# nv-legate/legate.sparse

Measured on AMD Instinct MI355X. Metric: cg_iters_per_sec, higher is better.
Workload: dtype fp64; 1 GPU; model=poisson2d-5pt-cg, nx=16384, n=268435456, nnz=1342111744, parallelism=dp1 1-D row partition + window gather

## Files before the change

sparse/kernels/__init__.py:

```python
from __future__ import annotations

import os

import torch

_EXT = None
_TRIED = False

_DIR = os.path.dirname(os.path.abspath(__file__))
BUILD_DIR = os.path.join(_DIR, "_build")
SO_PATH = os.path.join(BUILD_DIR, "sparse_hip.so")


def ext():
    global _EXT, _TRIED
    if _EXT is not None or _TRIED:
        return _EXT
    _TRIED = True
    if os.path.exists(SO_PATH):
        torch.ops.load_library(SO_PATH)
        _EXT = torch.ops.sparse_hip
    return _EXT


# ... 392 lines not shown
            and os.environ.get("SPARSE_DIA_NOCOMPRESS") != "1"):
        cvals = torch.zeros(W, dtype=dvals.dtype, device=A.device)
        mdt = (torch.uint8 if W <= 8 else
               torch.uint16 if W <= 16 else torch.uint32)
        mask = torch.empty(mp, dtype=mdt, device=A.device)
        ok = torch.ones(1, dtype=torch.int32, device=A.device)
        ext().dia_classify(dvals, cvals, mask, ok, W)
        if int(ok.item()):
            dvals = None
        else:
            cvals = mask = None
    ho = offs.tolist()
    adj = sum(1 << i for i in range(min(W, 32) - 1) if ho[i + 1] == ho[i] + 1)
    return DiaMirror(dvals, offs, W, m, row0, off_min=ho[0], off_max=ho[-1],
                     cvals=cvals, mask=mask, adj=adj)


def _pieces(p):
    hlo, own, hhi = p
    return hlo.contiguous(), own.contiguous(), hhi.contiguous()


def dia_spmv(dm: DiaMirror, pieces, y, col_lo: int, wsize: int,
             rbase: int = 0, rhi: int = -1):
    ext().dia_spmv(*dm.source(), dm.offs, *_pieces(pieces), y, dm.W, dm.m,
                   int(col_lo), dm.row0, int(wsize), int(rbase), int(rhi),
                   dm.adj)


def dia_spmv_dot(dm: DiaMirror, pieces, y, p, col_lo: int, wsize: int,
                 rbase: int = 0, rhi: int = -1):
    return ext().dia_spmv_dot(*dm.source(), dm.offs, *_pieces(pieces), y, p,
                              dm.W, dm.m, int(col_lo), dm.row0, int(wsize),
                              int(rbase), int(rhi), dm.adj)


def dia_spmv_bpdot(dm: DiaMirror, r_pieces, p_pieces, pnew, q,
                   beta_num, beta_den, col_lo: int, wsize: int):
    return ext().dia_spmv_bpdot(*dm.source(), dm.offs, *_pieces(r_pieces),
                                *_pieces(p_pieces), pnew, q, beta_num,
                                beta_den, dm.W, dm.m, int(col_lo), dm.row0,
                                int(wsize), dm.adj)


def cg_xr_norm2(x, p, r, q, a, b, *, nt: int = -1):
    n = x.numel()
    if n == 0:
        return torch.zeros((), dtype=x.dtype, device=x.device)
    ept = max(1, 16 // x.element_size())
    blocks = (n // ept + 255) // 256 + 1
    partial = torch.empty(blocks, dtype=x.dtype, device=x.device)
    ext().cg_xr_norm2(x, p, r, q, a.to(x.dtype), b.to(x.dtype), partial,
                      int(nt))
    return partial.sum()


def dia_residual(dm: DiaMirror, pieces, b, y, col_lo: int, wsize: int,
# ... 144 lines not shown
```

sparse/kernels/src/common.h:

```cpp
#pragma once

#include <type_traits>

#include <hip/hip_runtime.h>

#include <ATen/ATen.h>
#include <ATen/Dispatch.h>
#include <ATen/hip/HIPContext.h>
#include <c10/util/complex.h>

#define SPARSE_CHECK_HIP(cmd)                                             \
  do {                                                                    \
    hipError_t e = (cmd);                                                 \
    TORCH_CHECK(e == hipSuccess, "HIP error: ", hipGetErrorString(e));    \
  } while (0)

constexpr int WAVE = 64;

__device__ __forceinline__ int64_t ub_i64(const int64_t* arr, int64_t n, int64_t key) {
  int64_t lo = 0, hi = n;
  while (lo < hi) {
    int64_t mid = (lo + hi) >> 1;
    if (arr[mid] <= key) lo = mid + 1; else hi = mid;
  }
// ... 71 lines not shown
    if (lane == 0) ws[n * NW + wid] = s;
  }
  __syncthreads();
  T s = ZeroOf<T>::value();
  if (threadIdx.x < N) {
    const T* w = ws + threadIdx.x * NW;
    s = ((w[0] + w[1]) + w[2]) + w[3];
  }
  return s;
}

inline hipStream_t cur_stream() {
  return c10::hip::getCurrentHIPStreamMasqueradingAsCUDA().stream();
}

template <typename T>
__device__ __forceinline__ T nt_load(const T* __restrict__ p) {
  if constexpr (std::is_arithmetic_v<T>) {
    return __builtin_nontemporal_load(p);
  } else {
    return *p;
  }
}
```

sparse/kernels/src/elemwise.hip:

```cpp
#include "common.h"

namespace {

template <typename index_t>
__global__ void add_nnz_kernel(const int64_t* __restrict__ aip,
                               const index_t* __restrict__ aix,
                               const int64_t* __restrict__ bip,
                               const index_t* __restrict__ bix,
                               int64_t* __restrict__ out, int64_t m) {
  int64_t r = (int64_t)blockIdx.x * blockDim.x + threadIdx.x;
  if (r >= m) return;
  int64_t pa = aip[r], ea = aip[r + 1];
  int64_t pb = bip[r], eb = bip[r + 1];
  int64_t c = 0;
  while (pa < ea && pb < eb) {
    index_t ca = aix[pa], cb = bix[pb];
    if (ca == cb) { ++pa; ++pb; }
    else if (ca < cb) ++pa;
    else ++pb;
    ++c;
  }
  out[r] = c + (ea - pa) + (eb - pb);
}

// ... 98 lines not shown
    static_assert(sizeof(VVec<T>) == 16, "non-temporal path moves 16 bytes");
    const u32x4_t t =
        __builtin_nontemporal_load(reinterpret_cast<const u32x4_t*>(p));
    VVec<T> v;
    __builtin_memcpy(&v, &t, 16);
    return v;
  } else {
    return *p;
  }
}

template <bool NT, typename T>
__device__ __forceinline__ void vec_store(VVec<T>* p, const VVec<T>& v) {
  if constexpr (NT) {
    static_assert(sizeof(VVec<T>) == 16, "non-temporal path moves 16 bytes");
    u32x4_t t;
    __builtin_memcpy(&t, &v, 16);
    __builtin_nontemporal_store(t, reinterpret_cast<u32x4_t*>(p));
  } else {
    *p = v;
  }
}

enum : int { NT_NONE = 0, NT_READS = 1, NT_ALL = 2 };

template <typename T, bool ISALPHA, bool NEG, int NT>
__global__ __launch_bounds__(256) void axpby_kernel(
    T* __restrict__ y, const T* __restrict__ x, const T* __restrict__ a,
    const T* __restrict__ b, int64_t n) {
  constexpr int EPT = EptOf<T>::value;
  T s = (*a) / (*b);
  if (NEG) s = -s;
  const int64_t nv = n / EPT;
  const int64_t i = (int64_t)blockIdx.x * blockDim.x + threadIdx.x;
  if (i < nv) {
    auto* y2 = reinterpret_cast<VVec<T>*>(y);
    auto* x2 = reinterpret_cast<const VVec<T>*>(x);
    VVec<T> yv = vec_load<NT == NT_ALL>(y2 + i);
    const VVec<T> xv = vec_load<NT != NT_NONE>(x2 + i);
#pragma unroll
    for (int j = 0; j < EPT; ++j) {
      yv.v[j] = ISALPHA ? (yv.v[j] + s * xv.v[j]) : (xv.v[j] + s * yv.v[j]);
    }
    vec_store<NT == NT_ALL>(y2 + i, yv);
  }
  if (blockIdx.x == 0 && threadIdx.x == 0) {
    for (int64_t t = nv * EPT; t < n; ++t) {
      y[t] = ISALPHA ? (y[t] + s * x[t]) : (x[t] + s * y[t]);
    }
  }
}

constexpr int kStreamNtAuto = NT_ALL;
constexpr int64_t kStreamNtMinBytes = int64_t(256) << 20;

inline int stream_nt_mode(int64_t nt, int64_t vec_bytes, const char* who) {
  TORCH_CHECK(nt >= -1 && nt <= 2, who, ": nt must be -1, 0, 1 or 2, got ", nt);
  if (nt >= 0) return (int)nt;
  return vec_bytes >= kStreamNtMinBytes ? kStreamNtAuto : NT_NONE;
}

}

void add_nnz_hip(at::Tensor aip, at::Tensor aix, at::Tensor bip, at::Tensor bix,
                 at::Tensor out) {
  int64_t m = out.numel();
  if (m == 0) return;
  DISPATCH_INDEX(aix.scalar_type(), "add_nnz", [&] {
    hipLaunchKernelGGL((add_nnz_kernel<index_t>), dim3((m + 255) / 256), dim3(256),
                       0, cur_stream(), aip.data_ptr<int64_t>(),
                       aix.data_ptr<index_t>(), bip.data_ptr<int64_t>(),
                       bix.data_ptr<index_t>(), out.data_ptr<int64_t>(), m);
  });
  SPARSE_CHECK_HIP(hipGetLastError());
}

void add_compute_hip(at::Tensor aip, at::Tensor aix, at::Tensor av,
                     at::Tensor bip, at::Tensor bix, at::Tensor bv,
                     at::Tensor cip, at::Tensor cix, at::Tensor cv,
                     double alpha, double beta) {
  int64_t m = aip.numel() - 1;
  if (m == 0) return;
// ... 219 lines not shown
```

sparse/kernels/src/ops.cpp:

```cpp
#include <algorithm>

#include <torch/library.h>

#include <ATen/ATen.h>

void spmv_hip(at::Tensor, at::Tensor, at::Tensor, at::Tensor, at::Tensor,
              int64_t, double);
void spmv_dot_hip(at::Tensor, at::Tensor, at::Tensor, at::Tensor, at::Tensor,
                  at::Tensor, at::Tensor, int64_t);
void axpby_norm2_hip(at::Tensor, at::Tensor, at::Tensor, at::Tensor, bool,
                     bool, at::Tensor);
void build_ell_hip(at::Tensor, at::Tensor, at::Tensor, at::Tensor, at::Tensor,
                   int64_t, int64_t);
void build_dia_hip(at::Tensor, at::Tensor, at::Tensor, at::Tensor, at::Tensor,
                   int64_t, int64_t);
void ell_spmv_plain_hip(at::Tensor, at::Tensor, at::Tensor, at::Tensor,
                        at::Tensor, at::Tensor, int64_t, int64_t, int64_t,
                        int64_t, int64_t);
at::Tensor ell_spmv_dot_hip(at::Tensor, at::Tensor, at::Tensor, at::Tensor,
                            at::Tensor, at::Tensor, at::Tensor, int64_t,
                            int64_t, int64_t, int64_t, int64_t);
void ell_jacobi_hip(at::Tensor, at::Tensor, at::Tensor, at::Tensor,
                    at::Tensor, at::Tensor, at::Tensor, at::Tensor,
                    at::Tensor, int64_t, int64_t, int64_t, double);
void cg_xr_norm2_hip(at::Tensor, at::Tensor, at::Tensor, at::Tensor,
                     at::Tensor, at::Tensor, at::Tensor, int64_t);
using OptTensor = c10::optional<at::Tensor>;
void dia_classify_hip(at::Tensor, at::Tensor, at::Tensor, at::Tensor, int64_t);
at::Tensor dia_spmv_bpdot_hip(at::Tensor, OptTensor, at::Tensor, at::Tensor,
                              at::Tensor, at::Tensor, at::Tensor, at::Tensor,
                              at::Tensor, at::Tensor, at::Tensor, at::Tensor,
                              at::Tensor, int64_t, int64_t, int64_t, int64_t,
                              int64_t, int64_t);
void dia_spmv_plain_hip(at::Tensor, OptTensor, at::Tensor, at::Tensor,
                        at::Tensor, at::Tensor, at::Tensor, int64_t, int64_t,
                        int64_t, int64_t, int64_t, int64_t, int64_t, int64_t);
at::Tensor dia_spmv_dot_hip(at::Tensor, OptTensor, at::Tensor, at::Tensor,
                            at::Tensor, at::Tensor, at::Tensor, at::Tensor,
                            int64_t, int64_t, int64_t, int64_t, int64_t,
                            int64_t, int64_t, int64_t);
void dia_residual_hip(at::Tensor, OptTensor, at::Tensor, at::Tensor,
                      at::Tensor, at::Tensor, at::Tensor, at::Tensor, int64_t,
                      int64_t, int64_t, int64_t, int64_t, int64_t, int64_t,
                      int64_t);
void dia_jacobi_hip(at::Tensor, OptTensor, at::Tensor, at::Tensor, at::Tensor,
                    at::Tensor, at::Tensor, at::Tensor, at::Tensor,
                    at::Tensor, int64_t, int64_t, int64_t, int64_t, int64_t,
                    double, int64_t, int64_t, int64_t);
void add_nnz_hip(at::Tensor, at::Tensor, at::Tensor, at::Tensor, at::Tensor);
void add_compute_hip(at::Tensor, at::Tensor, at::Tensor, at::Tensor, at::Tensor,
                     at::Tensor, at::Tensor, at::Tensor, at::Tensor, double,
                     double);
void mult_nnz_hip(at::Tensor, at::Tensor, at::Tensor, at::Tensor, at::Tensor);
void mult_compute_hip(at::Tensor, at::Tensor, at::Tensor, at::Tensor,
                      at::Tensor, at::Tensor, at::Tensor, at::Tensor,
                      at::Tensor);
void mult_dense_hip(at::Tensor, at::Tensor, at::Tensor, at::Tensor, at::Tensor);
void axpby_hip(at::Tensor, at::Tensor, at::Tensor, at::Tensor, bool, bool,
               int64_t);
void spmm_hip(at::Tensor, at::Tensor, at::Tensor, at::Tensor, at::Tensor,
              int64_t);
void rspmm_hip(at::Tensor, at::Tensor, at::Tensor, at::Tensor, at::Tensor);
void bsr_spmm_hip(at::Tensor, at::Tensor, at::Tensor, at::Tensor, at::Tensor,
// ... 144 lines not shown
        "Tensor offs, Tensor(a!) dvals, int W, int row0) -> ()");
  m.def("ell_spmv(Tensor eidx, Tensor evals, Tensor hlo, Tensor own, "
        "Tensor hhi, Tensor(a!) y, int W, int m, int col_lo, "
        "int rbase, int rhi) -> ()");
  m.def("ell_spmv_dot(Tensor eidx, Tensor evals, Tensor hlo, Tensor own, "
        "Tensor hhi, Tensor(a!) y, Tensor pvec, int W, int m, int col_lo, "
        "int rbase, int rhi) -> Tensor");
  m.def("ell_jacobi(Tensor eidx, Tensor evals, Tensor hlo, Tensor own, "
        "Tensor hhi, Tensor xloc, Tensor b, Tensor dinv, Tensor(a!) xout, "
        "int W, int m, int col_lo, float omega) -> ()");
  m.def("cg_xr_norm2(Tensor(a!) x, Tensor p, Tensor(b!) r, Tensor q, "
        "Tensor a, Tensor b, Tensor(c!) dot_out, int nt=-1) -> ()");
  m.def("dia_classify(Tensor dvals, Tensor(a!) cvals, Tensor(b!) mask, "
        "Tensor(c!) ok, int W) -> ()");
  m.def("dia_spmv_bpdot(Tensor planes, Tensor? mask, Tensor offs, "
        "Tensor r_hlo, Tensor r_own, "
        "Tensor r_hhi, Tensor p_hlo, Tensor p_own, Tensor p_hhi, "
        "Tensor(a!) pnew, Tensor(b!) q, Tensor beta_num, Tensor beta_den, "
        "int W, int m, int col_lo, int row0, int wsize, int adj=0) "
        "-> Tensor");
  m.def("dia_spmv(Tensor planes, Tensor? mask, Tensor offs, Tensor hlo, "
        "Tensor own, "
        "Tensor hhi, Tensor(a!) y, int W, int m, int col_lo, int row0, "
        "int wsize, int rbase, int rhi, int adj=0) -> ()");
  m.def("dia_spmv_dot(Tensor planes, Tensor? mask, Tensor offs, Tensor hlo, "
        "Tensor own, "
        "Tensor hhi, Tensor(a!) y, Tensor pvec, int W, int m, int col_lo, "
        "int row0, int wsize, int rbase, int rhi, int adj=0) -> Tensor");
  m.def("dia_residual(Tensor planes, Tensor? mask, Tensor offs, Tensor hlo, "
        "Tensor own, "
        "Tensor hhi, Tensor b, Tensor(a!) y, int W, int m, int col_lo, "
        "int row0, int wsize, int rbase, int rhi, int adj=0) -> ()");
  m.def("dia_jacobi(Tensor planes, Tensor? mask, Tensor offs, Tensor hlo, "
        "Tensor own, "
        "Tensor hhi, Tensor xloc, Tensor b, Tensor dinv, Tensor(a!) xout, "
        "int W, int m, int col_lo, int row0, int wsize, float omega, "
        "int rbase, int rhi, int adj=0) -> ()");
  m.def("spmm(Tensor indptr, Tensor indices, Tensor vals, Tensor B, "
        "Tensor(a!) C, int col_lo) -> ()");
  m.def("rspmm(Tensor indptr, Tensor indices, Tensor vals, Tensor A, "
        "Tensor(a!) C) -> ()");
  m.def("bsr_spmm(Tensor bptr, Tensor bcol, Tensor bvals, Tensor B, "
        "Tensor(a!) C, int col_lo) -> ()");
  m.def("sddmm(Tensor indptr, Tensor indices, Tensor vals, Tensor C, "
        "Tensor D, Tensor(a!) out, int col_lo) -> ()");
  m.def("csr_to_dense(Tensor indptr, Tensor indices, Tensor vals, "
        "Tensor(a!) out) -> ()");
  m.def("coo_to_csr(Tensor rows, Tensor cols, Tensor vals, Tensor(a!) cursor, "
        "Tensor indptr, Tensor(b!) out_idx, Tensor(c!) out_vals, "
        "Tensor(d!) flags) -> ()");
  m.def("dense_to_csr(Tensor D, Tensor(a!) indptr_or_counts, "
// ... 71 lines not shown
```

sparse/kernels/src/spmv.hip:

```cpp
#include <type_traits>

#include "common.h"

namespace {

constexpr int BLK = 256;
constexpr int VT = 8;
constexpr int64_t NNZ_PER_BLOCK = (int64_t)BLK * VT;

template <typename U>
struct alignas(4 * sizeof(U) <= 16 ? 4 * sizeof(U) : 16) Quad {
  U v[4];
};

template <typename U>
struct alignas(2 * sizeof(U) <= 16 ? 2 * sizeof(U) : 16) Pair {
  U a, b;
};

template <typename T>
__device__ __forceinline__ void block_reduce_sum(T* red, int tid) {
  __syncthreads();
  for (int w = BLK / 2; w > 0; w >>= 1) {
    if (tid < w) red[tid] += red[tid + w];
// ... 377 lines not shown
struct DiaPlanes {
  static constexpr int kBatch = 1;
  const T* __restrict__ dvals;
  int64_t mp;

  struct Rows {
    const T* __restrict__ p;
    int64_t mp;
    __device__ __forceinline__ void at(int k, T& v0, T& v1) const {
      const int64_t base = (int64_t)k * mp;
      v0 = nt_load(&p[base]);
      v1 = nt_load(&p[base + 1]);
    }
  };
  __device__ __forceinline__ Rows rows(int64_t r0) const {
    return {dvals + r0, mp};
  }
};

template <int BYTES> struct UIntOf;
template <> struct UIntOf<2> { using type = uint16_t; };
template <> struct UIntOf<4> { using type = uint32_t; };
template <> struct UIntOf<8> { using type = uint64_t; };

template <typename T, typename M>
struct DiaConstPlanes {
  static constexpr int kBatch = 8;
  const T* __restrict__ cvals;
  const M* __restrict__ mask;

  struct Rows {
    const T* __restrict__ c;
    uint32_t m0, m1;
    __device__ __forceinline__ void at(int k, T& v0, T& v1) const {
      const T ck = c[k];
      const uint32_t bit = 1u << k;
      v0 = (m0 & bit) ? ck : T(0);
      v1 = (m1 & bit) ? ck : T(0);
    }
  };
  __device__ __forceinline__ Rows rows(int64_t r0) const {
    using M2 = typename UIntOf<2 * sizeof(M)>::type;
    const M2 w = nt_load(reinterpret_cast<const M2*>(&mask[r0]));
    return {cvals, (uint32_t)(M)w, (uint32_t)(w >> (8 * sizeof(M)))};
  }
};
// ... 32 lines not shown
        if (k + j < W) xpair(cbase + offs[k + j], x0[j], x1[j]);
      }
#pragma unroll
      for (int j = 0; j < U; ++j) {
        if (k + j < W) {
          T v0, v1;
          rows.at(k + j, v0, v1);
          a0 = fmadd(v0, x0[j], a0);
          a1 = fmadd(v1, x1[j], a1);
        }
      }
    }
  }
}

template <typename T>
__device__ __forceinline__ void store_pair_or_tail(T* __restrict__ dst,
                                                   int64_t r0, int64_t m,
                                                   int64_t rhi, T v0, T v1) {
  if (r0 + 1 < min(m, rhi)) {
    *reinterpret_cast<Pair<T>*>(&dst[r0]) = Pair<T>{v0, v1};
  } else if (r0 < m) {
    dst[r0] = v0;
  }
}

template <typename T>
__device__ __forceinline__ void jacobi_update(
    const T* __restrict__ xloc, const T* __restrict__ b,
    const T* __restrict__ dinv, T* __restrict__ xout, T omega, int64_t r0,
    int64_t m, int64_t rhi, T a0, T a1) {
  if (r0 + 1 < min(m, rhi)) {
    const Pair<T> xv = *reinterpret_cast<const Pair<T>*>(&xloc[r0]);
    const Pair<T> bv = *reinterpret_cast<const Pair<T>*>(&b[r0]);
    const Pair<T> dv = *reinterpret_cast<const Pair<T>*>(&dinv[r0]);
    *reinterpret_cast<Pair<T>*>(&xout[r0]) =
        Pair<T>{fmadd(omega * dv.a, bv.a - a0, xv.a),
                fmadd(omega * dv.b, bv.b - a1, xv.b)};
  } else if (r0 < m) {
    xout[r0] = fmadd(omega * dinv[r0], b[r0] - a0, xloc[r0]);
  }
}

template <typename T>
__device__ __forceinline__ void block_dot_partial(T d,
                                                  T* __restrict__ dot_partial) {
// ... 110 lines not shown
      x0 = fmadd(beta, p0v, r0v);
      x1 = fmadd(beta, p1v, r1v);
    };
    const int64_t cbase = row0 + r0 - col_lo;
    dia_accumulate(planes, offs, W, r0, cbase, pnew_pair, a0, a1);
    pnew_pair(cbase, p0, p1);
    store_pair_or_tail(pnew, r0, m, m, p0, p1);
    store_pair_or_tail(q, r0, m, m, a0, a1);
  }
  T d = ZeroOf<T>::value();
  if (r0 < m) d = fmadd(a0, p0, d);
  if (r0 + 1 < m) d = fmadd(a1, p1, d);
  block_dot_partial(d, dot_partial);
}

constexpr int kDiaPairs = 4;
constexpr int kDiaSmoothPairs = 2;
constexpr int kDiaBpdotPairs = 1;

constexpr int dia_spmv_pairs(int WC, bool resid) {
  return (!resid && WC >= 1 && WC <= 5) ? kDiaPairs : kDiaSmoothPairs;
}

template <int CTRL, typename T>
__device__ __forceinline__ T lane_shift(T v) {
  static_assert(sizeof(T) % 4 == 0, "whole dwords expected");
  int w[sizeof(T) / 4];
  __builtin_memcpy(w, &v, sizeof(T));
#pragma unroll
  for (int i = 0; i < (int)(sizeof(T) / 4); ++i) {
    w[i] = __builtin_amdgcn_update_dpp(w[i], w[i], CTRL, 0xf, 0xf, false);
  }
  __builtin_memcpy(&v, w, sizeof(T));
  return v;
}
template <typename T>
__device__ __forceinline__ T lane_above(T v) {
  return lane_shift<0x130>(v);
}
template <typename T>
__device__ __forceinline__ T lane_below(T v) {
  return lane_shift<0x138>(v);
}

enum DiaSrc { kDiaLoad, kDiaLoadAligned, kDiaFromLo, kDiaFromHi };

template <uint32_t ADJ>
struct DiaRun {
  static constexpr int start = ADJ ? __builtin_ctz(ADJ) : 0;
  static constexpr int len = ADJ ? __builtin_popcount(ADJ) + 1 : 1;
  static_assert(ADJ == 0 || (ADJ >> start) + 1 == (1u << (len - 1)),
                "the adjacent diagonals must form one run");
  __host__ __device__ static constexpr DiaSrc src(int P, int i) {
    const int q = i - start;
    if (ADJ == 0 || P < 0 || q < 0 || q >= len) return kDiaLoad;
    if (((P + q) & 1) == 0) return kDiaLoadAligned;
    return q > 0 ? kDiaFromLo : kDiaFromHi;
  }
  __host__ __device__ static constexpr bool two(int P, int i) {
    return src(P, i) == kDiaFromHi && len >= 3;
  }
};

template <int WC, int R, int NWIN, uint32_t ADJ, int P, typename T,
          typename M, typename Comb, typename Pre, typename Post>
__device__ __forceinline__ void dia_const_interior(
    const DiaConstPlanes<T, M>& planes, const int64_t* __restrict__ offs,
    int W, const T* const* own, Comb comb, bool ctr, int64_t rb,
    int64_t cb, int64_t (&o)[WC ? WC : 8], T (&c)[WC ? WC : 8], Pre pre,
    Post post) {
  constexpr int KB = WC ? WC : 8;
  using Run = DiaRun<ADJ>;
  using M2 = typename UIntOf<2 * sizeof(M)>::type;
  const int64_t t2 = 2 * (int64_t)threadIdx.x;
  const int lane = threadIdx.x & 63;
  M2 mw[R];
#pragma unroll
  for (int j = 0; j < R; ++j) {
    mw[j] = nt_load(
        reinterpret_cast<const M2*>(planes.mask + rb + t2 + j * 2 * BLK));
  }
  T a[R][2];
  Pair<T> cx[R];
#pragma unroll
  for (int j = 0; j < R; ++j) {
    a[j][0] = a[j][1] = ZeroOf<T>::value();
    cx[j] = Pair<T>{T(0), T(0)};
  }
  for (int k0 = 0; k0 < W; k0 += KB) {
    if (k0 > 0) {
#pragma unroll
      for (int i = 0; i < KB; ++i) {
        if (k0 + i < W) {
          o[i] = offs[k0 + i];
          c[i] = planes.cvals[k0 + i];
        }
      }
    }
    T xv[NWIN][R][KB][2];
#pragma unroll
    for (int i = 0; i < KB; ++i) {
      if (k0 + i < W) {
        const DiaSrc src = Run::src(P, i);
#pragma unroll
        for (int w = 0; w < NWIN; ++w) {
          const T* ub = own[w] + (cb + o[i]);
          const bool aligned =
              src == kDiaLoadAligned ||
              (reinterpret_cast<uintptr_t>(ub) % sizeof(Pair<T>)) == 0;
#pragma unroll
          for (int j = 0; j < R; ++j) {
            const T* p = ub + t2 + j * 2 * BLK;
            if (src == kDiaFromHi) {
              if (lane == 0 || (Run::two(P, i) && lane == 63)) {
                xv[w][j][i][0] = p[lane == 0 ? 0 : 3];
              }
            } else if (src == kDiaFromLo) {
              if (!(i >= 2 && Run::two(P, i - 2)) && lane == 63) {
                xv[w][j][i][0] = p[1];
              }
            } else if (aligned) {
              const Pair<T> t = *reinterpret_cast<const Pair<T>*>(p);
              xv[w][j][i][0] = t.a;
              xv[w][j][i][1] = t.b;
            } else {
              xv[w][j][i][0] = p[0];
              xv[w][j][i][1] = p[1];
            }
          }
        }
      }
    }
    if (k0 == 0) {
#pragma unroll
      for (int j = 0; j < R; ++j) pre(j, rb + t2 + j * 2 * BLK, true, ctr);
      __builtin_amdgcn_sched_barrier(0);
    }
    if (ADJ != 0 && P >= 0) {
#pragma unroll
      for (int w = 0; w < NWIN; ++w) {
#pragma unroll
        for (int j = 0; j < R; ++j) {
          T edge[KB];
#pragma unroll
          for (int i = 0; i < KB; ++i) {
            edge[i] = xv[w][j][i][0];
            if (Run::src(P, i) == kDiaFromLo) {
              const bool shared = i >= 2 && Run::two(P, i - 2);
              const T e = shared ? edge[i >= 2 ? i - 2 : 0] : edge[i];
              const T up = lane_above(xv[w][j][i > 0 ? i - 1 : 0][0]);
              xv[w][j][i][0] = xv[w][j][i > 0 ? i - 1 : 0][1];
              xv[w][j][i][1] = lane == 63 ? e : up;
            } else if (Run::src(P, i) == kDiaFromHi) {
              const T dn = lane_below(xv[w][j][i + 1 < KB ? i + 1 : i][1]);
              xv[w][j][i][1] = xv[w][j][i + 1 < KB ? i + 1 : i][0];
              xv[w][j][i][0] = lane == 0 ? edge[i] : dn;
            }
          }
        }
      }
    }
    if (WC > 0 && ctr) {
#pragma unroll
      for (int j = 0; j < R; ++j) {
        cx[j] = Pair<T>{xv[0][j][(KB - 1) / 2][0], xv[0][j][(KB - 1) / 2][1]};
      }
    }
#pragma unroll
    for (int j = 0; j < R; ++j) {
      const uint32_t m0 = (uint32_t)(M)mw[j];
      const uint32_t m1 = (uint32_t)(mw[j] >> (8 * sizeof(M)));
#pragma unroll
      for (int i = 0; i < KB; ++i) {
        if (k0 + i < W) {
          T v0[NWIN], v1[NWIN];
#pragma unroll
          for (int w = 0; w < NWIN; ++w) {
            v0[w] = xv[w][j][i][0];
            v1[w] = xv[w][j][i][1];
          }
          const uint32_t bit = 1u << (k0 + i);
          a[j][0] = fmadd((m0 & bit) ? c[i] : T(0), comb(v0), a[j][0]);
          a[j][1] = fmadd((m1 & bit) ? c[i] : T(0), comb(v1), a[j][1]);
        }
      }
    }
  }
#pragma unroll
  for (int j = 0; j < R; ++j) {
    post(j, rb + t2 + j * 2 * BLK, a[j][0], a[j][1], true, ctr, cx[j]);
  }
}

template <int WC, int R, bool SINGLE, int NWIN, uint32_t ADJ, typename T,
          typename M, typename Comb, typename Pre, typename Post>
__device__ __forceinline__ void dia_const_rows(
    const DiaConstPlanes<T, M>& planes, const int64_t* __restrict__ offs,
    int Wrt, const XWindow<T>& win0, const XWindow<T>& win1, Comb comb,
    const T* rowvec, int64_t m, int64_t row0, int64_t col_lo, int64_t rbase,
    int64_t rhi, Pre pre, Post post) {
  constexpr int KB = WC ? WC : 8;
  constexpr int64_t S = 2 * (int64_t)BLK * R;
  static_assert(ADJ == 0 || (WC > 0 && (ADJ >> (KB - 1)) == 0),
                "a plan needs a compile-time W");
  using Run = DiaRun<ADJ>;
  const int W = WC ? WC : Wrt;
  const int64_t lim = min(m, rhi);
  const int64_t rb = rbase + (int64_t)blockIdx.x * S;
  const int64_t cb = row0 + rb - col_lo - win0.nlo;
  const int64_t own_end = min(win0.nown, win0.wsize - win0.nlo);
  int64_t o[KB];
  T c[KB];
#pragma unroll
  for (int i = 0; i < KB; ++i) {
    if (i < W) {
      o[i] = offs[i];
      c[i] = planes.cvals[i];
    }
  }
  bool interior = rb + S <= lim && cb + o[0] >= 0 &&
                  cb + (S - 1) + (WC ? o[KB - 1] : offs[W - 1]) < own_end;
#pragma unroll
  for (int q = 1; q < Run::len; ++q) {
    interior = interior && o[Run::start + q] == o[Run::start] + q;
  }
  if (interior) {
    const T* own[NWIN];
    own[0] = win0.own;
    own[NWIN - 1] = (NWIN == 2 ? win1 : win0).own;
    const bool ctr = WC > 0 && NWIN == 1 && rowvec != nullptr &&
                     rowvec + rb == win0.own + cb && o[(KB - 1) / 2] == 0;
    auto body = [&](auto par) {
      dia_const_interior<WC, R, NWIN, ADJ, decltype(par)::value>(
          planes, offs, W, own, comb, ctr, rb, cb, o, c, pre, post);
    };
    if (ADJ == 0) {
      body(std::integral_constant<int, -1>{});
    } else {
      const T* u0 = own[0] + (cb + o[Run::start]);
      const T* u1 = own[NWIN - 1] + (cb + o[Run::start]);
      const bool un0 = reinterpret_cast<uintptr_t>(u0) % sizeof(Pair<T>) != 0;
      const bool un1 = reinterpret_cast<uintptr_t>(u1) % sizeof(Pair<T>) != 0;
      if (un0 != un1) {
        body(std::integral_constant<int, -1>{});
      } else if (un0) {
        body(std::integral_constant<int, 1>{});
      } else {
        body(std::integral_constant<int, 0>{});
      }
    }
  } else {
    const int64_t t2 = 2 * (int64_t)threadIdx.x;
#pragma unroll
    for (int j = 0; j < R; ++j) {
      const int64_t r0 = rb + t2 + j * 2 * BLK;
      if (r0 < rhi) {
        T a0 = ZeroOf<T>::value(), a1 = ZeroOf<T>::value();
        pre(j, r0, r0 + 1 < lim, false);
        dia_accumulate(
            planes, offs, W, r0, row0 + r0 - col_lo,
            [&](int64_t c0, T& x0, T& x1) {
              T v0[NWIN], v1[NWIN];
#pragma unroll
              for (int w = 0; w < NWIN; ++w) {
                (w == 0 ? win0 : win1)
                    .template pair<SINGLE, true>(c0, v0[w], v1[w]);
              }
              x0 = comb(v0);
              x1 = comb(v1);
            },
            a0, a1);
        post(j, r0, a0, a1, r0 + 1 < lim, false, Pair<T>{T(0), T(0)});
      }
    }
  }
}

template <typename T, typename M, int WC, uint32_t ADJ, bool FUSE_DOT,
          bool SINGLE, bool RESID>
__global__ __launch_bounds__(BLK) void dia_const_spmv_kernel(
    const DiaConstPlanes<T, M> planes, const int64_t* __restrict__ offs,
    const XWindow<T> win, T* __restrict__ y, const T* __restrict__ pvec,
    T* __restrict__ dot_partial, int64_t m, int W, int64_t col_lo,
    int64_t row0, int64_t rbase, int64_t rhi) {
  constexpr int R = dia_spmv_pairs(WC, RESID);
  const int64_t lim = min(m, rhi);
  Pair<T> pv[R];
  T d[R];
#pragma unroll
  for (int j = 0; j < R; ++j) {
    pv[j] = Pair<T>{T(0), T(0)};
    d[j] = T(0);
  }
  dia_const_rows<WC, R, SINGLE, 1, ADJ>(
      planes, offs, W, win, win, [](const T(&v)[1]) { return v[0]; },
      (FUSE_DOT || RESID) ? pvec : nullptr, m, row0, col_lo, rbase, rhi,
      [&](int j, int64_t r0, bool full, bool ctr) {
        if ((FUSE_DOT || RESID) && !ctr) {
          if (full) {
            pv[j] = *reinterpret_cast<const Pair<T>*>(&pvec[r0]);
          } else if (r0 < lim) {
            pv[j].a = pvec[r0];
          }
        }
      },
      [&](int j, int64_t r0, T a0, T a1, bool full, bool ctr, Pair<T> cx) {
        if (ctr) pv[j] = cx;
        if (RESID) {
          a0 = pv[j].a - a0;
          a1 = pv[j].b - a1;
        }
        if (full) {
          *reinterpret_cast<Pair<T>*>(&y[r0]) = Pair<T>{a0, a1};
        } else {
          store_pair_or_tail(y, r0, m, rhi, a0, a1);
        }
        if (FUSE_DOT) {
          T dd = T(0);
          if (full || r0 < lim) dd = fmadd(a0, pv[j].a, dd);
          if (full) dd = fmadd(a1, pv[j].b, dd);
          d[j] = dd;
        }
      });
  if (FUSE_DOT) {
    const T sum = block_sums_256<R>(d);
    const int64_t slot = (int64_t)blockIdx.x * R + threadIdx.x;
    if (threadIdx.x < R && slot * (2 * BLK) < rhi - rbase) {
      dot_partial[slot] = sum;
    }
  }
}

template <typename T, typename M, int WC, uint32_t ADJ, bool SINGLE>
__global__ __launch_bounds__(BLK) void dia_const_jacobi_kernel(
    const DiaConstPlanes<T, M> planes, const int64_t* __restrict__ offs,
    const XWindow<T> win, const T* __restrict__ xloc,
    const T* __restrict__ b, const T* __restrict__ dinv,
    T* __restrict__ xout, int64_t m, int W, int64_t col_lo, int64_t row0,
    T omega, int64_t rbase, int64_t rhi) {
  constexpr int R = kDiaSmoothPairs;
  Pair<T> xv[R], bv[R], dv[R];
  dia_const_rows<WC, R, SINGLE, 1, ADJ>(
      planes, offs, W, win, win, [](const T(&v)[1]) { return v[0]; }, xloc,
      m, row0, col_lo, rbase, rhi,
      [&](int j, int64_t r0, bool full, bool ctr) {
        if (full) {
          if (!ctr) xv[j] = *reinterpret_cast<const Pair<T>*>(&xloc[r0]);
          bv[j] = *reinterpret_cast<const Pair<T>*>(&b[r0]);
          dv[j] = *reinterpret_cast<const Pair<T>*>(&dinv[r0]);
        }
      },
      [&](int j, int64_t r0, T a0, T a1, bool full, bool ctr, Pair<T> cx) {
        if (ctr) xv[j] = cx;
        if (full) {
          *reinterpret_cast<Pair<T>*>(&xout[r0]) =
              Pair<T>{fmadd(omega * dv[j].a, bv[j].a - a0, xv[j].a),
                      fmadd(omega * dv[j].b, bv[j].b - a1, xv[j].b)};
        } else {
          jacobi_update(xloc, b, dinv, xout, omega, r0, m, rhi, a0, a1);
        }
      });
}

template <typename T, typename M, int WC, uint32_t ADJ, bool SINGLE>
__global__ __launch_bounds__(BLK) void dia_const_bpdot_kernel(
    const DiaConstPlanes<T, M> planes, const int64_t* __restrict__ offs,
    const XWindow<T> rwin, const XWindow<T> pwin, T* __restrict__ pnew,
    T* __restrict__ q, const T* __restrict__ beta_num,
    const T* __restrict__ beta_den, T* __restrict__ dot_partial, int64_t m,
    int64_t mp, int W, int64_t col_lo, int64_t row0) {
  constexpr int R = kDiaBpdotPairs;
  const T beta = (*beta_num) / (*beta_den);
  auto comb = [&](const T(&v)[2]) { return fmadd(beta, v[1], v[0]); };
  T rr[R][2], pp[R][2];
  T d[R];
#pragma unroll
  for (int j = 0; j < R; ++j) d[j] = T(0);
  dia_const_rows<WC, R, SINGLE, 2, ADJ>(
      planes, offs, W, rwin, pwin, comb, (const T*)nullptr, m, row0, col_lo,
      0, mp,
      [&](int j, int64_t r0, bool, bool) {
        const int64_t c0 = row0 + r0 - col_lo;
        rwin.template pair<SINGLE, true>(c0, rr[j][0], rr[j][1]);
        pwin.template pair<SINGLE, true>(c0, pp[j][0], pp[j][1]);
      },
      [&](int j, int64_t r0, T a0, T a1, bool full, bool, Pair<T>) {
        const T v0[2] = {rr[j][0], pp[j][0]}, v1[2] = {rr[j][1], pp[j][1]};
        const T p0 = comb(v0), p1 = comb(v1);
        if (full) {
          *reinterpret_cast<Pair<T>*>(&pnew[r0]) = Pair<T>{p0, p1};
          *reinterpret_cast<Pair<T>*>(&q[r0]) = Pair<T>{a0, a1};
        } else {
          store_pair_or_tail(pnew, r0, m, m, p0, p1);
          store_pair_or_tail(q, r0, m, m, a0, a1);
        }
        T dd = T(0);
        if (full || r0 < m) dd = fmadd(a0, p0, dd);
        if (full) dd = fmadd(a1, p1, dd);
        d[j] = dd;
      });
  const T sum = block_sums_256<R>(d);
// ... 260 lines not shown
  const RowPairLaunch L(evals.numel() / W, hlo, own, hhi, 0);
  if (L.empty()) return;
  DISPATCH_VALUES(evals.scalar_type(), "ell_jacobi", [&] {
    using T = scalar_t;
    DISPATCH_INDEX(eidx.scalar_type(), "ell_jacobi_idx", [&] {
      dispatch_bool(L.single, [&](auto single) {
        L.launch(ell_jacobi_kernel<T, index_t, decltype(single)::value>,
                 eidx.data_ptr<index_t>(), evals.data_ptr<T>(),
                 L.window<T>(hlo, own, hhi), xloc.data_ptr<T>(),
                 b.data_ptr<T>(), dinv.data_ptr<T>(), xout.data_ptr<T>(), m,
                 L.mp, W, col_lo, omega);
      });
    });
  });
}

template <bool RESID>
static at::Tensor dia_spmv_impl(const at::Tensor& planes, const OptTensor& mask,
                                const at::Tensor& offs, const at::Tensor& hlo,
                                const at::Tensor& own, const at::Tensor& hhi,
                                at::Tensor& y, const at::Tensor* pvec,
                                int64_t W, int64_t m, int64_t col_lo,
                                int64_t row0, int64_t wsize, int64_t rbase,
                                int64_t rhi, int64_t adj) {
  const RowPairLaunch L(dia_mp(planes, mask, W), hlo, own, hhi, wsize, rbase,
                        rhi);
  const bool fuse_dot = pvec && !RESID;
  at::Tensor partial;
  if (L.empty()) return partial;
  if (fuse_dot) partial = at::empty({L.nblocks}, planes.options());
  DISPATCH_VALUES(planes.scalar_type(), "dia_spmv", [&] {
    using T = scalar_t;
    dispatch_dia_planes<T>(planes, mask, W, [&](auto pl) {
      dispatch_bool(fuse_dot, [&](auto fuse) {
        dispatch_bool(L.single, [&](auto single) {
          using PL = decltype(pl);
          const T* pp = pvec ? pvec->data_ptr<T>() : nullptr;
          T* dp = fuse_dot ? partial.data_ptr<T>() : nullptr;
          if constexpr (RESID && decltype(fuse)::value) {
          } else if constexpr (DiaConstOf<PL>::value) {
            using M = typename DiaConstOf<PL>::mask_t;
            dispatch_dia_wc<M>(W, adj, [&](auto wc, auto plan) {
              L.launch_pairs<dia_spmv_pairs(decltype(wc)::value, RESID)>(
                  dia_const_spmv_kernel<T, M, decltype(wc)::value,
                                        decltype(plan)::value,
                                        decltype(fuse)::value,
                                        decltype(single)::value, RESID>,
                  pl, offs.data_ptr<int64_t>(), L.window<T>(hlo, own, hhi),
                  y.data_ptr<T>(), pp, dp, m, W, col_lo, row0, L.rbase,
                  L.rhi);
            });
          } else {
            L.launch(dia_spmv_kernel<T, PL, decltype(fuse)::value,
                                     decltype(single)::value, RESID>,
                     pl, offs.data_ptr<int64_t>(), L.window<T>(hlo, own, hhi),
                     y.data_ptr<T>(), pp, dp, m, L.mp, W, col_lo, row0,
                     L.rbase, L.rhi);
          }
        });
      });
    });
  });
  return partial;
}

void dia_spmv_plain_hip(at::Tensor planes, OptTensor mask, at::Tensor offs,
                        at::Tensor hlo, at::Tensor own, at::Tensor hhi,
                        at::Tensor y, int64_t W, int64_t m, int64_t col_lo,
                        int64_t row0, int64_t wsize, int64_t rbase,
                        int64_t rhi, int64_t adj) {
  dia_spmv_impl<false>(planes, mask, offs, hlo, own, hhi, y, nullptr, W, m,
                       col_lo, row0, wsize, rbase, rhi, adj);
}

at::Tensor dia_spmv_dot_hip(at::Tensor planes, OptTensor mask, at::Tensor offs,
                            at::Tensor hlo, at::Tensor own, at::Tensor hhi,
                            at::Tensor y, at::Tensor pvec, int64_t W,
                            int64_t m, int64_t col_lo, int64_t row0,
                            int64_t wsize, int64_t rbase, int64_t rhi,
                            int64_t adj) {
  return sum_or_zero(dia_spmv_impl<false>(planes, mask, offs, hlo, own, hhi, y,
                                          &pvec, W, m, col_lo, row0, wsize,
                                          rbase, rhi, adj),
                     planes);
}

void dia_residual_hip(at::Tensor planes, OptTensor mask, at::Tensor offs,
                      at::Tensor hlo, at::Tensor own, at::Tensor hhi,
                      at::Tensor b, at::Tensor y, int64_t W, int64_t m,
                      int64_t col_lo, int64_t row0, int64_t wsize,
                      int64_t rbase, int64_t rhi, int64_t adj) {
  dia_spmv_impl<true>(planes, mask, offs, hlo, own, hhi, y, &b, W, m, col_lo,
                      row0, wsize, rbase, rhi, adj);
}

void dia_jacobi_hip(at::Tensor planes, OptTensor mask, at::Tensor offs,
                    at::Tensor hlo, at::Tensor own, at::Tensor hhi,
                    at::Tensor xloc, at::Tensor b, at::Tensor dinv,
                    at::Tensor xout, int64_t W, int64_t m, int64_t col_lo,
                    int64_t row0, int64_t wsize, double omega, int64_t rbase,
                    int64_t rhi, int64_t adj) {
  const RowPairLaunch L(dia_mp(planes, mask, W), hlo, own, hhi, wsize, rbase,
                        rhi);
  if (L.empty()) return;
  DISPATCH_VALUES(planes.scalar_type(), "dia_jacobi", [&] {
    using T = scalar_t;
// ... 72 lines not shown
```

Measured before the change: 259.3 iters/s.

## Stage DIA mask and halo edges through LDS, add nontemporal y stores in SpMV

In the constant-plane DIA SpMV kernel, each thread now loads its mask row in one contiguous nontemporal load, shares it through LDS, and reads back the strided per-pair layout. Wave-boundary halo values are exchanged through shared memory, so only block-edge threads do extra global loads instead of every wave's edge lanes. A new nt knob (auto when the vector is 256MB or larger) selects nontemporal stores for y. The trade is an added __syncthreads, more LDS use and extra template instantiations, aimed at fewer and narrower global loads and less cache pollution.

New measurement: 262.8 iters/s, median of 6. No clear change (+1.4%).

```diff
diff --git a/sparse/kernels/__init__.py b/sparse/kernels/__init__.py
--- a/sparse/kernels/__init__.py
+++ b/sparse/kernels/__init__.py
@@ -438,17 +438,17 @@
 
 
 def dia_spmv(dm: DiaMirror, pieces, y, col_lo: int, wsize: int,
-             rbase: int = 0, rhi: int = -1):
+             rbase: int = 0, rhi: int = -1, *, nt: int = -1):
     ext().dia_spmv(*dm.source(), dm.offs, *_pieces(pieces), y, dm.W, dm.m,
                    int(col_lo), dm.row0, int(wsize), int(rbase), int(rhi),
-                   dm.adj)
+                   dm.adj, int(nt))
 
 
 def dia_spmv_dot(dm: DiaMirror, pieces, y, p, col_lo: int, wsize: int,
-                 rbase: int = 0, rhi: int = -1):
+                 rbase: int = 0, rhi: int = -1, *, nt: int = -1):
     return ext().dia_spmv_dot(*dm.source(), dm.offs, *_pieces(pieces), y, p,
                               dm.W, dm.m, int(col_lo), dm.row0, int(wsize),
-                              int(rbase), int(rhi), dm.adj)
+                              int(rbase), int(rhi), dm.adj, int(nt))
 
 
 def dia_spmv_bpdot(dm: DiaMirror, r_pieces, p_pieces, pnew, q,
diff --git a/sparse/kernels/src/common.h b/sparse/kernels/src/common.h
--- a/sparse/kernels/src/common.h
+++ b/sparse/kernels/src/common.h
@@ -117,3 +117,14 @@
     return *p;
   }
 }
+
+enum : int { NT_NONE = 0, NT_READS = 1, NT_ALL = 2 };
+
+constexpr int kStreamNtAuto = NT_ALL;
+constexpr int64_t kStreamNtMinBytes = int64_t(256) << 20;
+
+inline int stream_nt_mode(int64_t nt, int64_t vec_bytes, const char* who) {
+  TORCH_CHECK(nt >= -1 && nt <= 2, who, ": nt must be -1, 0, 1 or 2, got ", nt);
+  if (nt >= 0) return (int)nt;
+  return vec_bytes >= kStreamNtMinBytes ? kStreamNtAuto : NT_NONE;
+}
diff --git a/sparse/kernels/src/elemwise.hip b/sparse/kernels/src/elemwise.hip
--- a/sparse/kernels/src/elemwise.hip
+++ b/sparse/kernels/src/elemwise.hip
@@ -144,8 +144,6 @@
   }
 }
 
-enum : int { NT_NONE = 0, NT_READS = 1, NT_ALL = 2 };
-
 template <typename T, bool ISALPHA, bool NEG, int NT>
 __global__ __launch_bounds__(256) void axpby_kernel(
     T* __restrict__ y, const T* __restrict__ x, const T* __restrict__ a,
@@ -171,15 +169,6 @@
       y[t] = ISALPHA ? (y[t] + s * x[t]) : (x[t] + s * y[t]);
     }
   }
-}
-
-constexpr int kStreamNtAuto = NT_ALL;
-constexpr int64_t kStreamNtMinBytes = int64_t(256) << 20;
-
-inline int stream_nt_mode(int64_t nt, int64_t vec_bytes, const char* who) {
-  TORCH_CHECK(nt >= -1 && nt <= 2, who, ": nt must be -1, 0, 1 or 2, got ", nt);
-  if (nt >= 0) return (int)nt;
-  return vec_bytes >= kStreamNtMinBytes ? kStreamNtAuto : NT_NONE;
 }
 
 }
diff --git a/sparse/kernels/src/ops.cpp b/sparse/kernels/src/ops.cpp
--- a/sparse/kernels/src/ops.cpp
+++ b/sparse/kernels/src/ops.cpp
@@ -34,11 +34,12 @@
                               int64_t, int64_t);
 void dia_spmv_plain_hip(at::Tensor, OptTensor, at::Tensor, at::Tensor,
                         at::Tensor, at::Tensor, at::Tensor, int64_t, int64_t,
-                        int64_t, int64_t, int64_t, int64_t, int64_t, int64_t);
+                        int64_t, int64_t, int64_t, int64_t, int64_t, int64_t,
+                        int64_t);
 at::Tensor dia_spmv_dot_hip(at::Tensor, OptTensor, at::Tensor, at::Tensor,
                             at::Tensor, at::Tensor, at::Tensor, at::Tensor,
                             int64_t, int64_t, int64_t, int64_t, int64_t,
-                            int64_t, int64_t, int64_t);
+                            int64_t, int64_t, int64_t, int64_t);
 void dia_residual_hip(at::Tensor, OptTensor, at::Tensor, at::Tensor,
                       at::Tensor, at::Tensor, at::Tensor, at::Tensor, int64_t,
                       int64_t, int64_t, int64_t, int64_t, int64_t, int64_t,
@@ -229,11 +230,12 @@
   m.def("dia_spmv(Tensor planes, Tensor? mask, Tensor offs, Tensor hlo, "
         "Tensor own, "
         "Tensor hhi, Tensor(a!) y, int W, int m, int col_lo, int row0, "
-        "int wsize, int rbase, int rhi, int adj=0) -> ()");
+        "int wsize, int rbase, int rhi, int adj=0, int nt=-1) -> ()");
   m.def("dia_spmv_dot(Tensor planes, Tensor? mask, Tensor offs, Tensor hlo, "
         "Tensor own, "
         "Tensor hhi, Tensor(a!) y, Tensor pvec, int W, int m, int col_lo, "
-        "int row0, int wsize, int rbase, int rhi, int adj=0) -> Tensor");
+        "int row0, int wsize, int rbase, int rhi, int adj=0, int nt=-1) "
+        "-> Tensor");
   m.def("dia_residual(Tensor planes, Tensor? mask, Tensor offs, Tensor hlo, "
         "Tensor own, "
         "Tensor hhi, Tensor b, Tensor(a!) y, int W, int m, int col_lo, "
diff --git a/sparse/kernels/src/spmv.hip b/sparse/kernels/src/spmv.hip
--- a/sparse/kernels/src/spmv.hip
+++ b/sparse/kernels/src/spmv.hip
@@ -423,6 +423,14 @@
 template <> struct UIntOf<2> { using type = uint16_t; };
 template <> struct UIntOf<4> { using type = uint32_t; };
 template <> struct UIntOf<8> { using type = uint64_t; };
+template <int BYTES> struct UIntAlign2;
+template <> struct UIntAlign2<2> { typedef uint16_t type; };
+template <> struct UIntAlign2<4> {
+  typedef uint32_t type __attribute__((aligned(2)));
+};
+template <> struct UIntAlign2<8> {
+  typedef uint64_t type __attribute__((aligned(2)));
+};
 
 template <typename T, typename M>
 struct DiaConstPlanes {
@@ -501,6 +509,16 @@
     *reinterpret_cast<Pair<T>*>(&dst[r0]) = Pair<T>{v0, v1};
   } else if (r0 < m) {
     dst[r0] = v0;
+  }
+}
+
+template <bool NT, typename T>
+__device__ __forceinline__ void store_pair(T* __restrict__ dst, T v0, T v1) {
+  if constexpr (NT) {
+    typedef T vec2 __attribute__((ext_vector_type(2)));
+    __builtin_nontemporal_store(vec2{v0, v1}, reinterpret_cast<vec2*>(dst));
+  } else {
+    *reinterpret_cast<Pair<T>*>(dst) = Pair<T>{v0, v1};
   }
 }
 
@@ -657,6 +675,12 @@
   return (!resid && WC >= 1 && WC <= 5) ? kDiaPairs : kDiaSmoothPairs;
 }
 
+enum : int { kDiaLdsMask = 1, kDiaLdsEdges = 2 };
+constexpr int kDiaSpmvLds = kDiaLdsMask | kDiaLdsEdges;
+constexpr int dia_spmv_lds(int WC, bool resid) {
+  return (!resid && WC >= 1 && WC <= 5) ? kDiaSpmvLds : 0;
+}
+
 template <int CTRL, typename T>
 __device__ __forceinline__ T lane_shift(T v) {
   static_assert(sizeof(T) % 4 == 0, "whole dwords expected");
@@ -697,23 +721,45 @@
   }
 };
 
-template <int WC, int R, int NWIN, uint32_t ADJ, int P, typename T,
+
+template <int WC, int R, int NWIN, uint32_t ADJ, int P, int LDSX, typename T,
           typename M, typename Comb, typename Pre, typename Post>
 __device__ __forceinline__ void dia_const_interior(
     const DiaConstPlanes<T, M>& planes, const int64_t* __restrict__ offs,
     int W, const T* const* own, Comb comb, bool ctr, int64_t rb,
     int64_t cb, int64_t (&o)[WC ? WC : 8], T (&c)[WC ? WC : 8], Pre pre,
-    Post post) {
+    Post post, unsigned char* lmask, T* ledge) {
   constexpr int KB = WC ? WC : 8;
   using Run = DiaRun<ADJ>;
   using M2 = typename UIntOf<2 * sizeof(M)>::type;
+  static_assert(LDSX == 0 || (WC > 0 && sizeof(M) == 1 && R >= 2),
+                "LDS staging: compile-time W, u8 mask, R >= 2");
+  constexpr bool LMASK = (LDSX & kDiaLdsMask) != 0;
+  constexpr bool LEDGE = (LDSX & kDiaLdsEdges) != 0 && ADJ != 0 && P >= 0;
+  constexpr int NRUN = R * (BLK / WAVE);
+  constexpr int S = 2 * BLK * R;
   const int64_t t2 = 2 * (int64_t)threadIdx.x;
   const int lane = threadIdx.x & 63;
+  const int wid = threadIdx.x / WAVE;
+  using MRow = typename UIntOf<LMASK ? 2 * R : 2>::type;
+  auto lfirst = [&](int w, int s, int g) -> T& {
+    return ledge[(w * KB + s) * NRUN + g];
+  };
+  auto llast = [&](int w, int s, int g) -> T& {
+    return ledge[((NWIN + w) * KB + s) * NRUN + g];
+  };
   M2 mw[R];
-#pragma unroll
-  for (int j = 0; j < R; ++j) {
-    mw[j] = nt_load(
-        reinterpret_cast<const M2*>(planes.mask + rb + t2 + j * 2 * BLK));
+  MRow mrow = 0;
+  if constexpr (LMASK) {
+    mrow = __builtin_nontemporal_load(
+        reinterpret_cast<const typename UIntAlign2<sizeof(MRow)>::type*>(
+            planes.mask + rb + 2 * R * (int64_t)threadIdx.x));
+  } else {
+#pragma unroll
+    for (int j = 0; j < R; ++j) {
+      mw[j] = nt_load(
+          reinterpret_cast<const M2*>(planes.mask + rb + t2 + j * 2 * BLK));
+    }
   }
   T a[R][2];
   Pair<T> cx[R];
@@ -733,6 +779,7 @@
       }
     }
     T xv[NWIN][R][KB][2];
+    T bedge[NWIN][KB];
 #pragma unroll
     for (int i = 0; i < KB; ++i) {
       if (k0 + i < W) {
@@ -743,10 +790,22 @@
           const bool aligned =
               src == kDiaLoadAligned ||
               (reinterpret_cast<uintptr_t>(ub) % sizeof(Pair<T>)) == 0;
+          bedge[w][i] = T(0);
+          if (LEDGE && src == kDiaFromHi) {
+            if (threadIdx.x == 0 ||
+                (Run::two(P, i) && threadIdx.x == BLK - 1)) {
+              bedge[w][i] = ub[threadIdx.x == 0 ? 0 : S + 1];
+            }
+          } else if (LEDGE && src == kDiaFromLo) {
+            if (!(i >= 2 && Run::two(P, i - 2)) && threadIdx.x == BLK - 1) {
+              bedge[w][i] = ub[S - 1];
+            }
+          }
 #pragma unroll
           for (int j = 0; j < R; ++j) {
             const T* p = ub + t2 + j * 2 * BLK;
-            if (src == kDiaFromHi) {
+            if (LEDGE && (src == kDiaFromHi || src == kDiaFromLo)) {
+            } else if (src == kDiaFromHi) {
               if (lane == 0 || (Run::two(P, i) && lane == 63)) {
                 xv[w][j][i][0] = p[lane == 0 ? 0 : 3];
               }
@@ -771,6 +830,36 @@
       for (int j = 0; j < R; ++j) pre(j, rb + t2 + j * 2 * BLK, true, ctr);
       __builtin_amdgcn_sched_barrier(0);
     }
+    if constexpr (LDSX != 0) {
+      if constexpr (LMASK) {
+        *reinterpret_cast<MRow*>(lmask + sizeof(MRow) * threadIdx.x) = mrow;
+      }
+      if constexpr (LEDGE) {
+#pragma unroll
+        for (int w = 0; w < NWIN; ++w) {
+#pragma unroll
+          for (int s = 0; s < KB; ++s) {
+            const bool first =
+                s + 1 < KB && Run::src(P, s + 1) == kDiaFromLo;
+            const bool last = s >= 1 && Run::src(P, s - 1) == kDiaFromHi;
+#pragma unroll
+            for (int j = 0; j < R; ++j) {
+              const int g = j * (BLK / WAVE) + wid;
+              if (first && lane == 0) lfirst(w, s, g) = xv[w][j][s][0];
+              if (last && lane == 63) llast(w, s, g) = xv[w][j][s][1];
+            }
+          }
+        }
+      }
+      __syncthreads();
+      if constexpr (LMASK) {
+#pragma unroll
+        for (int j = 0; j < R; ++j) {
+          mw[j] = *reinterpret_cast<const M2*>(lmask + 2 * threadIdx.x +
+                                               j * 2 * BLK);
+        }
+      }
+    }
     if (ADJ != 0 && P >= 0) {
 #pragma unroll
       for (int w = 0; w < NWIN; ++w) {
@@ -779,17 +868,31 @@
           T edge[KB];
 #pragma unroll
           for (int i = 0; i < KB; ++i) {
-            edge[i] = xv[w][j][i][0];
+            const bool shared = i >= 2 && Run::two(P, i - 2);
+            T elo, ehi;
+            if constexpr (LEDGE) {
+              const int g = j * (BLK / WAVE) + wid;
+              elo = ehi = edge[i] = T(0);
+              if (Run::src(P, i) == kDiaFromLo) {
+                const T nb = lfirst(w, i > 0 ? i - 1 : 0, min(g + 1, NRUN - 1));
+                ehi = g + 1 < NRUN ? nb : bedge[w][shared ? i - 2 : i];
+              } else if (Run::src(P, i) == kDiaFromHi) {
+                const T nb = llast(w, i + 1 < KB ? i + 1 : i, max(g - 1, 0));
+                elo = g > 0 ? nb : bedge[w][i];
+              }
+            } else {
+              edge[i] = xv[w][j][i][0];
+              elo = edge[i];
+              ehi = shared ? edge[i >= 2 ? i - 2 : 0] : edge[i];
+            }
             if (Run::src(P, i) == kDiaFromLo) {
-              const bool shared = i >= 2 && Run::two(P, i - 2);
-              const T e = shared ? edge[i >= 2 ? i - 2 : 0] : edge[i];
               const T up = lane_above(xv[w][j][i > 0 ? i - 1 : 0][0]);
               xv[w][j][i][0] = xv[w][j][i > 0 ? i - 1 : 0][1];
-              xv[w][j][i][1] = lane == 63 ? e : up;
+              xv[w][j][i][1] = lane == 63 ? ehi : up;
             } else if (Run::src(P, i) == kDiaFromHi) {
               const T dn = lane_below(xv[w][j][i + 1 < KB ? i + 1 : i][1]);
               xv[w][j][i][1] = xv[w][j][i + 1 < KB ? i + 1 : i][0];
-              xv[w][j][i][0] = lane == 0 ? edge[i] : dn;
+              xv[w][j][i][0] = lane == 0 ? elo : dn;
             }
           }
         }
@@ -827,8 +930,8 @@
   }
 }
 
-template <int WC, int R, bool SINGLE, int NWIN, uint32_t ADJ, typename T,
-          typename M, typename Comb, typename Pre, typename Post>
+template <int WC, int R, bool SINGLE, int NWIN, uint32_t ADJ, int LDSX,
+          typename T, typename M, typename Comb, typename Pre, typename Post>
 __device__ __forceinline__ void dia_const_rows(
     const DiaConstPlanes<T, M>& planes, const int64_t* __restrict__ offs,
     int Wrt, const XWindow<T>& win0, const XWindow<T>& win1, Comb comb,
@@ -860,14 +963,18 @@
     interior = interior && o[Run::start + q] == o[Run::start] + q;
   }
   if (interior) {
+    constexpr bool LE = (LDSX & kDiaLdsEdges) != 0 && ADJ != 0;
+    __shared__ __align__(16) unsigned char lmask[(LDSX & kDiaLdsMask) ? S : 16];
+    __shared__ T ledge[LE ? 2 * NWIN * KB * R * (BLK / WAVE) : 1];
     const T* own[NWIN];
     own[0] = win0.own;
     own[NWIN - 1] = (NWIN == 2 ? win1 : win0).own;
     const bool ctr = WC > 0 && NWIN == 1 && rowvec != nullptr &&
                      rowvec + rb == win0.own + cb && o[(KB - 1) / 2] == 0;
     auto body = [&](auto par) {
-      dia_const_interior<WC, R, NWIN, ADJ, decltype(par)::value>(
-          planes, offs, W, own, comb, ctr, rb, cb, o, c, pre, post);
+      dia_const_interior<WC, R, NWIN, ADJ, decltype(par)::value, LDSX>(
+          planes, offs, W, own, comb, ctr, rb, cb, o, c, pre, post, lmask,
+          ledge);
     };
     if (ADJ == 0) {
       body(std::integral_constant<int, -1>{});
@@ -912,7 +1019,7 @@
 }
 
 template <typename T, typename M, int WC, uint32_t ADJ, bool FUSE_DOT,
-          bool SINGLE, bool RESID>
+          bool SINGLE, bool RESID, int LDSX = 0, bool NTY = false>
 __global__ __launch_bounds__(BLK) void dia_const_spmv_kernel(
     const DiaConstPlanes<T, M> planes, const int64_t* __restrict__ offs,
     const XWindow<T> win, T* __restrict__ y, const T* __restrict__ pvec,
@@ -927,7 +1034,7 @@
     pv[j] = Pair<T>{T(0), T(0)};
     d[j] = T(0);
   }
-  dia_const_rows<WC, R, SINGLE, 1, ADJ>(
+  dia_const_rows<WC, R, SINGLE, 1, ADJ, LDSX>(
       planes, offs, W, win, win, [](const T(&v)[1]) { return v[0]; },
       (FUSE_DOT || RESID) ? pvec : nullptr, m, row0, col_lo, rbase, rhi,
       [&](int j, int64_t r0, bool full, bool ctr) {
@@ -946,7 +1053,7 @@
           a1 = pv[j].b - a1;
         }
         if (full) {
-          *reinterpret_cast<Pair<T>*>(&y[r0]) = Pair<T>{a0, a1};
+          store_pair<NTY>(&y[r0], a0, a1);
         } else {
           store_pair_or_tail(y, r0, m, rhi, a0, a1);
         }
@@ -975,7 +1082,7 @@
     T omega, int64_t rbase, int64_t rhi) {
   constexpr int R = kDiaSmoothPairs;
   Pair<T> xv[R], bv[R], dv[R];
-  dia_const_rows<WC, R, SINGLE, 1, ADJ>(
+  dia_const_rows<WC, R, SINGLE, 1, ADJ, 0>(
       planes, offs, W, win, win, [](const T(&v)[1]) { return v[0]; }, xloc,
       m, row0, col_lo, rbase, rhi,
       [&](int j, int64_t r0, bool full, bool ctr) {
@@ -1011,7 +1118,7 @@
   T d[R];
 #pragma unroll
   for (int j = 0; j < R; ++j) d[j] = T(0);
-  dia_const_rows<WC, R, SINGLE, 2, ADJ>(
+  dia_const_rows<WC, R, SINGLE, 2, ADJ, 0>(
       planes, offs, W, rwin, pwin, comb, (const T*)nullptr, m, row0, col_lo,
       0, mp,
       [&](int j, int64_t r0, bool, bool) {
@@ -1318,10 +1425,12 @@
                                 at::Tensor& y, const at::Tensor* pvec,
                                 int64_t W, int64_t m, int64_t col_lo,
                                 int64_t row0, int64_t wsize, int64_t rbase,
-                                int64_t rhi, int64_t adj) {
+                                int64_t rhi, int64_t adj, int64_t nt = 0) {
   const RowPairLaunch L(dia_mp(planes, mask, W), hlo, own, hhi, wsize, rbase,
                         rhi);
   const bool fuse_dot = pvec && !RESID;
+  const bool nty =
+      stream_nt_mode(nt, y.numel() * y.element_size(), "dia_spmv") == NT_ALL;
   at::Tensor partial;
   if (L.empty()) return partial;
   if (fuse_dot) partial = at::empty({L.nblocks}, planes.options());
@@ -1337,14 +1446,18 @@
           } else if constexpr (DiaConstOf<PL>::value) {
             using M = typename DiaConstOf<PL>::mask_t;
             dispatch_dia_wc<M>(W, adj, [&](auto wc, auto plan) {
-              L.launch_pairs<dia_spmv_pairs(decltype(wc)::value, RESID)>(
-                  dia_const_spmv_kernel<T, M, decltype(wc)::value,
-                                        decltype(plan)::value,
-                                        decltype(fuse)::value,
-                                        decltype(single)::value, RESID>,
-                  pl, offs.data_ptr<int64_t>(), L.window<T>(hlo, own, hhi),
-                  y.data_ptr<T>(), pp, dp, m, W, col_lo, row0, L.rbase,
-                  L.rhi);
+              dispatch_bool(nty && !RESID, [&](auto ntc) {
+                constexpr int WC = decltype(wc)::value;
+                L.launch_pairs<dia_spmv_pairs(WC, RESID)>(
+                    dia_const_spmv_kernel<T, M, WC, decltype(plan)::value,
+                                          decltype(fuse)::value,
+                                          decltype(single)::value, RESID,
+                                          dia_spmv_lds(WC, RESID),
+                                          decltype(ntc)::value && !RESID>,
+                    pl, offs.data_ptr<int64_t>(), L.window<T>(hlo, own, hhi),
+                    y.data_ptr<T>(), pp, dp, m, W, col_lo, row0, L.rbase,
+                    L.rhi);
+              });
             });
           } else {
             L.launch(dia_spmv_kernel<T, PL, decltype(fuse)::value,
@@ -1364,9 +1477,9 @@
                         at::Tensor hlo, at::Tensor own, at::Tensor hhi,
                         at::Tensor y, int64_t W, int64_t m, int64_t col_lo,
                         int64_t row0, int64_t wsize, int64_t rbase,
-                        int64_t rhi, int64_t adj) {
+                        int64_t rhi, int64_t adj, int64_t nt) {
   dia_spmv_impl<false>(planes, mask, offs, hlo, own, hhi, y, nullptr, W, m,
-                       col_lo, row0, wsize, rbase, rhi, adj);
+                       col_lo, row0, wsize, rbase, rhi, adj, nt);
 }
 
 at::Tensor dia_spmv_dot_hip(at::Tensor planes, OptTensor mask, at::Tensor offs,
@@ -1374,10 +1487,10 @@
                             at::Tensor y, at::Tensor pvec, int64_t W,
                             int64_t m, int64_t col_lo, int64_t row0,
                             int64_t wsize, int64_t rbase, int64_t rhi,
-                            int64_t adj) {
+                            int64_t adj, int64_t nt) {
   return sum_or_zero(dia_spmv_impl<false>(planes, mask, offs, hlo, own, hhi, y,
                                           &pvec, W, m, col_lo, row0, wsize,
-                                          rbase, rhi, adj),
+                                          rbase, rhi, adj, nt),
                      planes);
 }
 
```
